# kuboyoo/alphazero-general-ori

Measured on AMD Instinct MI355X. Metric: self-play rollouts/sec (32k boards, 2p Splendor) at 1/2/4/8 MI355X, higher is better.
Workload: dtype fp32 (network) / int8 (boards) / f64 (tree statistics)

## Files before the change

### alphazero-general-ori_amd/csrc/mcts.hip

```cpp
#include <hip/hip_runtime.h>

#include <cmath>
#include <cstring>
#include <new>

#include "../../include/splendor_amd.h"

#include "board_phases.h"
#include "mcts_device.h"
#include "nn_stage.h"
#include "spl_ctx.h"

using namespace spl;

#ifndef SPL_BOUNDS_CHECK
#define SPL_BOUNDS_CHECK 0
#endif
#if SPL_BOUNDS_CHECK
__device__ unsigned long long g_bounds[4 + 64];
__device__ __noinline__ void bounds_note(int site, long long v, int t) {
    atomicAdd(&g_bounds[4 + (site & 63)], 1ull);
    if (atomicAdd(&g_bounds[0], 1ull) == 0) {
        g_bounds[1] = (unsigned long long)v; g_bounds[2] = (unsigned long long)site; g_bounds[3] = (unsigned long long)t;
    }
// ... 270 lines not shown
    for (int j = 0; j < (ec + 63) / 64; j++) {
        const int i = 64 * j + l;
        const double g = i < ec ? det_gamma(C.dir_alpha, C.seed, gb, stream, (uint32_t)i * 4096u) : 0.0;
        if (gbuf && i < ec) gbuf[i] = g;
        const int m = min(64, ec - 64 * j);
        const int lo = __double2loint(g), hi = __double2hiint(g);
        for (int k = 0; k < m; k++)
            acc = acc + __hiloint2double(__builtin_amdgcn_readlane(hi, k), __builtin_amdgcn_readlane(lo, k));
    }
    const bool ok = acc > 0.0;
    const double inv = ok ? 1.0 / acc : 0.0;
#pragma unroll 1
    for (int j = 0; j < (ec + 63) / 64; j++) {
        const int i = 64 * j + l;
        if (i < ec) {
            const int a = action_at(bits, i);
            const double g = gbuf ? gbuf[i] : (ok ? det_gamma(C.dir_alpha, C.seed, gb, stream, (uint32_t)i * 4096u) : 0.0);
            const double d = ok ? g * inv : 1.0 / (double)ec;
            pr[a] = (float)(0.75 * (double)pr[a] + 0.25 * d);
        }
    }
    wave_lds_fence();
    const float nsum = wave_np_sum409(pr);
    for (int a = l; a < SPL_ACTIONS; a += 64)
        if ((bits[a >> 6] >> (a & 63)) & 1) pr[a] = pr[a] / nsum;
    wave_lds_fence();
}

struct RunScr {
    uint64_t bits[7];
    float pr[416];
    float cp[SPL_ACTIONS];
    int16_t ca[SPL_ACTIONS];
    int16_t cvi[SPL_ACTIONS];
};

__device__ int noise_kept_root(const Pools &P, const SearchCfg &C, int t, const NodeRun &r, uint32_t stream,
                               uint64_t *bits, float *pr, float *cp, int16_t *ca, int16_t *cvi, double *gbuf = nullptr,
                               int gcap = 0) {
    const int l = lane_id();
    run_bits(P, r, bits);
    for (int a = l; a < 416; a += 64) pr[a] = 0.f;
    wave_lds_fence();
    for (int i = l; i < r.ec; i += 64) {
        const EdgeP e = *P.ep(r.eb + i);
        pr[e.a] = e.p;
        const int k = order_of(bits, e.a);
        ca[k] = e.a;
        cvi[k] = e.vi;
    }
    wave_lds_fence();
    root_noise_lds(C, t, stream, pr, bits, r.ec, gbuf, gcap);
    wave_lds_fence();
    for (int k = l; k < r.ec; k += 64) cp[k] = pr[ca[k]];
    wave_lds_fence();
    return write_sorted_run(P, r.eb, r.vb, r.ec, cp, ca, cvi);
}
__device__ __forceinline__ int noise_kept_root(const Pools &P, const SearchCfg &C, int t, const NodeRun &r,
                                               uint32_t stream, RunScr &S) {
    return noise_kept_root(P, C, t, r, stream, S.bits, S.pr, S.cp, S.ca, S.cvi);
}

#ifndef SPL_HOME_N
#define SPL_HOME_N 32
#endif
#ifndef SPL_HOME_E
#define SPL_HOME_E 24
#endif
__device__ __forceinline__ int pop_page(int32_t *stack, int32_t *top) {
    const int k = atomicSub(top, 1);
    if (k <= 0) { atomicAdd(top, 1); return -1; }
    return stack[k - 1];
}

__device__ int node_slot(const Pools &P, TreeHdr *H, int t, int id, int *npg_reg = nullptr) {
    if (id >= P.nmax) return -1;
    const int pi = id >> NPG_SHIFT;
    int32_t *tab = P.ntab + (size_t)t * P.nptab;
    if (pi >= (npg_reg ? *npg_reg : H->npg)) {
        const int pg = pi < P.nhome ? t * P.nhome + pi : pop_page(P.nfree, P.alloc + 0);
        if (pg < 0) { atomicAdd(P.alloc + 2, 1); return -1; }
        tab[pi] = pg;
        P.npidx[pg] = pi;
        H->npg = pi + 1;
        if (npg_reg) *npg_reg = pi + 1;
        return pg * NPG + (id & (NPG - 1));
    }
    return node_g(P, t, id);
}

struct AllocState {
    int64_t enext;
    int eleft, epg, edge_count;
};
__device__ __forceinline__ AllocState alloc_state(const TreeHdr *H) { return AllocState{H->enext, H->eleft, H->epg, H->edge_count}; }
__device__ int64_t unit_alloc_s(const Pools &P, TreeHdr *H, int t, int n, AllocState &a) {
    if (a.eleft < n) {
        if (a.epg >= P.eptab) return -1;
        const int pg = a.epg < P.ehome ? t * P.ehome + a.epg : pop_page(P.efree, P.alloc + 1);
        if (pg < 0) { atomicAdd(P.alloc + 3, 1); return -1; }
        P.etab[(size_t)t * P.eptab + a.epg] = pg;
        P.epidx[pg] = a.epg;
        a.epg += 1;
        H->epg = a.epg;
        a.enext = (int64_t)pg * UPG;
        a.eleft = UPG;
    }
    const int64_t b = a.enext;
    a.enext = b + n; a.eleft -= n; a.edge_count += n;
    H->enext = a.enext; H->eleft = a.eleft; H->edge_count = a.edge_count;
    return b;
}

__device__ __forceinline__ void push_pages(int32_t *stack, int32_t *top, int cap, const int32_t *tab, int from, int to,
                                           int home) {
    from = max(from, home);
    const int n = to - from;
    const int32_t *src = tab + from;
    if (n <= 0) return;
    int base = 0;
    if (lane_id() == 0) base = atomicAdd(top, n);
    base = __shfl(base, 0, 64);
    for (int i = lane_id(); i < n; i += 64)
        if (base + i < cap) stack[base + i] = src[i];
}

struct GcScr {
    int64_t *ost;
    int64_t *ovb;
    uint64_t *buf;
    int32_t *remap;
    int32_t *nvs;
    int32_t *cs;
    int32_t *cnt;
    int32_t *inv;
    int32_t *queue;
    int32_t *oec;
    int32_t *own;
};
__host__ __device__ inline size_t gc_ints(int nmax, int emax) {
    return 11 * (size_t)(nmax + 2) + 3 * (size_t)emax + 64;
}
__device__ __forceinline__ GcScr gc_scr(int32_t *base, int nmax, int emax) {
    const size_t m = (size_t)nmax + 2;
    GcScr S;
    S.ost = reinterpret_cast<int64_t *>(base);
    S.ovb = reinterpret_cast<int64_t *>(base + 2 * m);
    S.buf = reinterpret_cast<uint64_t *>(base + 4 * m);
    int32_t *q = base + 4 * m + 2 * (size_t)emax;
    S.remap = q; S.nvs = q + m; S.cs = q + 2 * m; S.cnt = q + 3 * m;
    S.inv = q + 4 * m; S.queue = q + 5 * m; S.oec = q + 6 * m; S.own = q + 7 * m;
    return S;
}

__device__ void mark_linked(const Pools &P, int t, int rootl, int32_t *mark, int32_t *q) {
    const int l = lane_id();
    const int nc = P.hdr[t].node_count;
    for (int i = l; i < nc; i += 64) mark[i] = i == rootl ? 1 : 0;
    if (l == 0) q[0] = rootl;
    wave_lds_fence();
    int head = 0, tail = 1;
    while (head < tail) {
        const int nbt = min(64, tail - head);
        int64_t vb = 0;
        int cnt = 0;
        if (l < nbt) {
            const int g = node_g(P, t, q[head + l]);
            if (!P.nd[g].h.term) {
                const NodeCold c = P.nd[g].c;
                vb = c.vb();
                cnt = c.vcnt();
            }
        }
        head += nbt;
        int incl = cnt;
#pragma unroll
        for (int o = 1; o < 64; o <<= 1) {
            const int y = __shfl_up(incl, o, 64);
            if (l >= o) incl += y;
        }
        const int tot = __shfl(incl, 63, 64), excl = incl - cnt;
        for (int c0 = 0; c0 < tot; c0 += 64) {
            const int e = c0 + l;
            int lo = 0;
#pragma unroll
            for (int step = 32; step > 0; step >>= 1)
                if (__shfl(excl, lo + step, 64) <= e) lo += step;
            const int64_t vbo = __shfl(vb, lo, 64);
            const int exo = __shfl(excl, lo, 64);
            const int c = e < tot ? P.vr(vbo + REC_UNITS * (e - exo))->child : -1;
            BCHK(c < 0 || IN_TREE(P, t, c, nc), 58, c, t, (void)0);
            const int cl = c >= 0 ? node_l(P, c) : -1;
            const bool fresh = cl >= 0 && atomicCAS(&mark[cl], 0, 1) == 0;
            const uint64_t bm = __ballot(fresh);
            if (fresh) q[tail + __popcll(bm & lanemask_lt())] = cl;
            tail += __popcll(bm);
            wave_lds_fence();
        }
    }
}

typedef uint32_t u32x4 __attribute__((ext_vector_type(4)));

constexpr int GCT = 512, GCW8 = GCT / 64;
struct GcLds {
    int32_t wsum[GCW8];
    int32_t bc[4];
};
__device__ __forceinline__ int block_scan(int x, int &total, GcLds &L) {
    const int l = lane_id(), w = threadIdx.x >> 6;
    int incl = x;
#pragma unroll
    for (int o = 1; o < 64; o <<= 1) {
        const int y = __shfl_up(incl, o, 64);
        if (l >= o) incl += y;
    }
    if (l == 63) L.wsum[w] = incl;
    __syncthreads();
    int off = 0, tot = 0;
#pragma unroll
    for (int i = 0; i < GCW8; i++) {
        const int v = L.wsum[i];
        off += i < w ? v : 0;
        tot += v;
    }
    __syncthreads();
    total = tot;
    return off + incl - x;
}

#ifndef GC_PROBE
#define GC_PROBE 0
#endif
#if GC_PROBE
constexpr int GC_WG_MAX_PROBE = 1024;
__device__ unsigned long long g_gc_probe[GC_WG_MAX_PROBE][16];
__device__ unsigned long long g_gc_probe_max[GC_WG_MAX_PROBE][8];
#define GPROBE(k)                                                                 \
    if (threadIdx.x == 0) {                                                       \
        const uint64_t c_ = __builtin_readcyclecounter();                         \
        gacc[k] += c_ - glast;                                                    \
        glast = c_;                                                               \
    }
#else
#define GPROBE(k)
#endif
constexpr int GC_NOFIT = -2;
#ifndef GC_SR
#define GC_SR 8
#endif
#ifndef GC_CR
#define GC_CR 4
#endif
template <int CR = 4>
__device__ int compact_tree(const Pools &P, int t, int root, int root_round, const GcScr &S, GcLds &L,
                            int bunits, bool linked = false) {
    const int tid = threadIdx.x;
    TreeHdr *H = P.hdr + t;
    const int nc = H->node_count;
    const int rootl = root >= 0 ? node_l(P, root) : -1;
    int32_t *remap = S.remap;
#if GC_PROBE
    uint64_t gacc[8] = {0, 0, 0, 0, 0, 0, 0, 0}, glast = __builtin_readcyclecounter();
    const uint64_t gstart = glast;
#endif
    if (linked) {
        if (tid < 64) mark_linked(P, t, rootl, remap, S.queue);
        __syncthreads();
    }
    int kept = 0;
    for (int base = 0; base < nc; base += GCT) {
        const int i = base + tid;
        bool keep = false;
        if (i < nc) keep = i == rootl || (linked ? remap[i] == 1 : P.nd[node_g(P, t, i)].h.round > root_round);
        int tot;
        const int ex = block_scan(keep ? 1 : 0, tot, L);
        if (i < nc) remap[i] = keep ? kept + ex : -1;
        kept += tot;
    }
    __syncthreads();
    GPROBE(0)
    for (int i = tid; i < nc; i += GCT) {
        int sz = -1;
        if (remap[i] >= 0) {
            sz = 0;
            const int g = node_g(P, t, i);
            const Node nd = P.nd[g];
            if (!nd.h.term) sz = nd.c.ec + REC_UNITS * nd.c.vcnt();
        }
        S.nvs[i] = sz;
    }
    __syncthreads();
    if (tid < 64) {
        const int l = tid;
        int run = 0;
        constexpr int PD = 4;
        int pre[PD];
#pragma unroll
        for (int d = 0; d < PD; d++) pre[d] = 64 * d + l < nc ? S.nvs[64 * d + l] : -1;
        for (int base = 0; base < nc; base += 64) {
            const int i = base + l;
            const int szk = pre[0];
#pragma unroll
            for (int d = 0; d + 1 < PD; d++) pre[d] = pre[d + 1];
            pre[PD - 1] = base + 64 * PD + l < nc ? S.nvs[base + 64 * PD + l] : -1;
            const bool kept = szk >= 0;
            const int sz = kept ? szk : 0;
            bool pending = sz > 0;
            int start = run;
            for (;;) {
                const int x = pending ? sz : 0;
                int incl = x;
#pragma unroll
                for (int o = 1; o < 64; o <<= 1) {
                    const int y = __shfl_up(incl, o, 64);
                    if (l >= o) incl += y;
                }
                const int st = run + incl - x;
                const bool strad = pending && (st & (UPG - 1)) + sz > UPG;
                const uint64_t m = __ballot(strad);
                if (!m) {
                    if (pending) start = st;
                    run += __shfl(incl, 63, 64);
                    break;
                }
                const int f = __ffsll((unsigned long long)m) - 1;
                if (pending && l < f) { start = st; pending = false; }
                run = (__builtin_amdgcn_readlane(st, f) & ~(UPG - 1)) + UPG;
            }
            if (kept) S.nvs[i] = start;
        }
        if (l == 0) L.bc[0] = run;
    }
    __syncthreads();
    const int run = L.bc[0];
    GPROBE(1)
    if (run > H->epg * UPG) return GC_NOFIT;
    __syncthreads();
    int my_units = 0;
    for (int base = 0; base < nc; base += GCT) {
        const int i = base + tid;
        const int ni = i < nc ? remap[i] : -1;
        uint64_t k0 = 0, k1 = 0;
        Node nd{};
        int vs = 0;
        if (ni >= 0) {
            const int g = node_g(P, t, i);
            k0 = P.nkey0[g]; k1 = P.nkey1[g];
            nd = P.nd[g];
            vs = S.nvs[i];
        }
        __syncthreads();
        if (ni >= 0) {
            const int ng = node_g(P, t, ni);
            const bool term = nd.h.term;
            const int ec = nd.c.ec, vcnt = term ? 0 : nd.c.vcnt();
            const int sz = term ? 0 : ec + REC_UNITS * vcnt;
            Node w = nd;
            S.queue[ni] = term ? -1 : nd.h.bchild;
            S.ost[ni] = nd.c.eb(); S.ovb[ni] = nd.c.vb(); S.oec[ni] = term ? 0 : ec;
            if (!term) {
                w.c.set_eb(ec > 0 ? unit_g(P, t, vs) : 0, vcnt);
                w.c.set_vb(vcnt > 0 ? unit_g(P, t, vs + ec) : 0, vcnt);
            }
            w.h.h2 = -1; w.h.h3 = -1;
            P.nkey0[ng] = k0; P.nkey1[ng] = k1;
            P.nd[ng] = w;
            S.cs[ni] = vs; S.cnt[ni] = sz; S.inv[ni] = i;
            my_units += sz;
        }
    }
    int units;
    (void)block_scan(my_units, units, L);
    GPROBE(2)
    for (int ni = tid; ni < kept; ni += GCT) {
        const int ch = S.queue[ni];
        if (ch >= 0) {
            BCHK(IN_TREE(P, t, ch, nc), 56, ((long long)ni << 32) | (uint32_t)ch, t, (void)0);
            const int nl = remap[node_l(P, ch)];
            P.nd[node_g(P, t, ni)].h.bchild = nl >= 0 ? node_g(P, t, nl) : -1;
            BCHK(nl < 0 || P.nd[node_g(P, t, nl)].h.round == P.nd[node_g(P, t, ni)].h.round + 1, 40,
                 ((long long)ni << 32) | (uint32_t)nl, t, (void)0);
        }
    }
    for (int k = tid; k < run; k += GCT) S.own[k] = -1;
    __syncthreads();
    for (int ni = tid; ni < kept; ni += GCT) {
        const int c0 = S.cs[ni], c = S.cnt[ni];
        for (int e = 0; e < c; e++) S.own[c0 + e] = ni;
    }
    __syncthreads();
    GPROBE(3)
    constexpr int SR = GC_SR;
    for (int k0 = 0; k0 < run; k0 += GCT * SR) {
        int j[SR];
#pragma unroll
        for (int r = 0; r < SR; r++) {
            const int k = k0 + GCT * r + tid;
            j[r] = k < run ? S.own[k] : -1;
        }
        int64_t src[SR];
        bool link[SR];
#pragma unroll
        for (int r = 0; r < SR; r++) {
            src[r] = 0; link[r] = false;
            if (j[r] >= 0) {
                const int rel = k0 + GCT * r + tid - S.cs[j[r]], ec = S.oec[j[r]];
                if (rel < ec) {
                    src[r] = S.ost[j[r]] + rel;
                } else {
                    const int rr = rel - ec;
                    src[r] = S.ovb[j[r]] + rr;
                    link[r] = rr % REC_UNITS == REC_LINK_UNIT;
                }
            }
        }
        uint64_t v[SR];
#pragma unroll
        for (int r = 0; r < SR; r++) v[r] = j[r] >= 0 ? P.eu[src[r]] : 0;
#pragma unroll
        for (int r = 0; r < SR; r++) {
            if (!link[r]) continue;
            const int ch = (int)(uint32_t)v[r];
            int nch = -1;
            if (ch >= 0) {
                BCHK(IN_TREE(P, t, ch, nc), 57, ((long long)j[r] << 32) | (uint32_t)ch, t, (void)0);
                const int nl = remap[node_l(P, ch)];
                if (nl >= 0) nch = node_g(P, t, nl);
                BCHK(nl < 0 || P.nd[nch].h.round == P.nd[node_g(P, t, j[r])].h.round + 1, 41,
                     ((long long)j[r] << 32) | (uint32_t)nl, t, (void)0);
            }
            v[r] = (v[r] & 0xFFFFFFFF00000000ull) | (uint64_t)(uint32_t)nch;
        }
#pragma unroll
        for (int r = 0; r < SR; r++)
            if (j[r] >= 0) S.buf[k0 + GCT * r + tid] = v[r];
    }
    __syncthreads();
    GPROBE(4)
    for (int k0 = 0; k0 < run; k0 += GCT * SR) {
        int j[SR];
        uint64_t v[SR];
#pragma unroll
        for (int r = 0; r < SR; r++) {
            const int k = k0 + GCT * r + tid;
            j[r] = k < run ? S.own[k] : -1;
            v[r] = k < run ? S.buf[k] : 0;
        }
#pragma unroll
        for (int r = 0; r < SR; r++)
            if (j[r] >= 0) P.eu[unit_g(P, t, k0 + GCT * r + tid)] = v[r];
    }
    if (P.nbrd) {
        u32x4 *bb = reinterpret_cast<u32x4 *>(P.nbrd);
        const int bu = kept * bunits;
        constexpr int R = 2 * CR;
        for (int k0 = 0; k0 < bu; k0 += GCT * R) {
            u32x4 d[R];
            size_t dst[R];
            bool mv[R];
#pragma unroll
            for (int r = 0; r < R; r++) {
                const int k = k0 + GCT * r + tid;
                mv[r] = false; dst[r] = 0; d[r] = u32x4{0, 0, 0, 0};
                if (k < bu) {
                    const int nn = k / bunits, u = k - nn * bunits, on = S.inv[nn];
                    if (on != nn) {
                        mv[r] = true;
                        dst[r] = (size_t)node_g(P, t, nn) * bunits + u;
                        d[r] = bb[(size_t)node_g(P, t, on) * bunits + u];
                    }
                }
            }
            __syncthreads();
#pragma unroll
            for (int r = 0; r < R; r++)
                if (mv[r]) bb[dst[r]] = d[r];
            __syncthreads();
        }
    }
    GPROBE(5)
    int32_t *hs = P.hslot + (size_t)t * P.hcap;
    for (int i = tid; i < P.hcap; i += GCT) hs[i] = -1;
    __syncthreads();
    for (int i = tid; i < kept; i += GCT) {
        const int g = node_g(P, t, i);
        const uint64_t k0 = P.nkey0[g];
        uint32_t h = (uint32_t)(k0 ^ (k0 >> 32)) & (uint32_t)(P.hcap - 1);
        while (atomicCAS(&hs[h], -1, g) != -1) h = (h + 1) & (uint32_t)(P.hcap - 1);
    }
    const int npg = (kept + NPG - 1) >> NPG_SHIFT, epg = (run + UPG - 1) >> UPG_SHIFT;
    const int onpg = H->npg, oepg = H->epg;
    const int nroot = rootl >= 0 && remap[rootl] >= 0 ? node_g(P, t, remap[rootl]) : -1;
    const int eleft = epg * UPG - run;
    const int64_t enext = eleft > 0 ? unit_g(P, t, run) : 0;
    __syncthreads();
    if (tid < 64) {
        push_pages(P.nfree, P.alloc + 0, P.npages, P.ntab + (size_t)t * P.nptab, npg, onpg, P.nhome);
        push_pages(P.efree, P.alloc + 1, P.epages, P.etab + (size_t)t * P.eptab, epg, oepg, P.ehome);
    }
    if (tid == 0) {
        H->node_count = kept; H->edge_count = units;
        H->npg = npg; H->epg = epg; H->eleft = eleft; H->enext = enext;
        H->live_gc = kept; H->units_gc = units; H->gcs += 1;
    }
    __syncthreads();
    GPROBE(6)
#if GC_PROBE
    if (tid == 0) {
        unsigned long long *g = g_gc_probe[blockIdx.x % GC_WG_MAX_PROBE];
        for (int k = 0; k < 7; k++) g[k] += gacc[k];
        g[8] += 1;
        const unsigned long long tot = glast - gstart;
        g[9] += tot;
        if (tot > g[10]) {
            g[10] = tot; g[11] = (unsigned long long)run; g[12] = (unsigned long long)kept; g[13] = (unsigned long long)nc;
            for (int k = 0; k < 7; k++) g_gc_probe_max[blockIdx.x % GC_WG_MAX_PROBE][k] = gacc[k];
        }
    }
#endif
    return nroot;
}

__device__ __forceinline__ long long units_used(const TreeHdr *H) { return (long long)H->epg * UPG - H->eleft; }
__device__ __forceinline__ bool tree_fits(const Pools &P, const SearchCfg &C, const TreeHdr *H) {
    return H->node_count + H->budget + 1 <= P.nmax &&
           units_used(H) + 4 * SPL_ACTIONS + (long long)H->budget * C.edge_reserve <= (long long)P.eptab * UPG;
}
__device__ void empty_tree(const Pools &P, int t) {
    TreeHdr *H = P.hdr + t;
    const int npg = H->npg, epg = H->epg;
    push_pages(P.nfree, P.alloc + 0, P.npages, P.ntab + (size_t)t * P.nptab, 0, npg, P.nhome);
    push_pages(P.efree, P.alloc + 1, P.epages, P.etab + (size_t)t * P.eptab, 0, epg, P.ehome);
    int32_t *hs = P.hslot + (size_t)t * P.hcap;
    if (H->node_count > 0 || npg > 0)
        for (int i = lane_id(); i < P.hcap; i += 64) hs[i] = -1;
    __builtin_amdgcn_wave_barrier();
    if (lane_id() == 0) {
        H->node_count = 0; H->edge_count = 0; H->npg = 0; H->epg = 0; H->eleft = 0; H->enext = 0;
        H->live_gc = 0; H->units_gc = 0;
    }
    __builtin_amdgcn_wave_barrier();
}
__device__ __forceinline__ void gc_push(const Pools &P, TreeHdr *H, int t) {
    if (H->gc_queued) return;
    H->gc_queued = 1;
    const int k = atomicAdd(&P.counters[2], 1);
    P.gcq[k] = t;
}

#ifndef GC_ALPHA_FREE
#define GC_ALPHA_FREE 8.f
#endif
template <int N>
__device__ void begin_search(const Pools &P, const SearchCfg &C, int t, const int8_t *s, bool keep,
                             bool force_full) {
    using Lx = Lay<N>;
    const int l = lane_id();
    TreeHdr *H = P.hdr + t;
    wave_store_board<N>(P.root_state + (size_t)t * Lx::S, s);
    const int mv = H->move_no;
    const bool full = force_full || philox_u01(C.seed, C.board_base + t, ST_FULL | (uint32_t)mv, 0) < C.prob_full;
    const int budget = full ? C.num_sims : C.num_sims / C.ratio_full;
    int root = -1, gcs = 0;
    const int rr = (uint8_t)bt(row(s, 0), 6);
    if (keep && H->node_count > 0) {
        uint64_t k0, k1;
        wave_fingerprint<N>(s, k0, k1);
        root = hash_lookup(P, t, k0, k1);
        BCHK(root < 0 || IN_TREE(P, t, root, H->node_count), 54, root, t, (void)0);
        const int nc = H->node_count;
        const long long used = units_used(H);
        const bool must = nc + budget + 1 > P.nmax ||
                          used + 4 * SPL_ACTIONS + (long long)budget * C.edge_reserve > (long long)P.eptab * UPG;
        const float f = fminf((float)P.alloc[0] / (float)max(P.npages - P.nhome * P.ntrees, 1),
                              (float)P.alloc[1] / (float)max(P.epages - P.ehome * P.ntrees, 1));
        const float alpha = f >= 0.75f ? GC_ALPHA_FREE : (f >= 0.5f ? 4.f : fmaxf(0.125f, 8.f * f));
        const bool should = nc > (int)((1.f + alpha) * (float)H->live_gc) + budget + NPG ||
                            used > (long long)((1.f + alpha) * (float)H->units_gc) +
                                       (long long)budget * C.edge_reserve + UPG;
        gcs = must || !C.selfplay ? 3 : (should ? 5 : 0);
    } else {
        empty_tree(P, t);
    }
    wave_lds_fence();
    if (l == 0) {
        H->root = root;
        H->sims_done = 0;
        H->full = full;
        H->budget = budget;
        H->forced = full && C.forced_playouts;
        H->noise_pending = full && C.dirichlet;
        H->leaf_kind = LEAF_NONE;
        H->overflow = 0;
        H->gc_state = gcs;
        H->root_round = rr;
        H->move_no = mv + 1;
        H->depth = 0;
        H->wd_search = 0;
        if (gcs) gc_push(P, H, t);
    }
    wave_lds_fence();
}

#ifndef GC_WG
#define GC_WG 256
#endif
#ifndef GC_SHOULD_CAP
#define GC_SHOULD_CAP GC_WG
#endif
template <int N>
__global__ __launch_bounds__(GCT) void k_gc(Pools P, SearchCfg C) {
    __shared__ GcLds L;
    __shared__ int keep_s;
    const int tid = threadIdx.x;
    const int tail = P.counters[2];
    const int ftail = P.counters[5];
    if (tail == 0 && ftail == 0) return;
    const GcScr S = gc_scr(P.gscr + (size_t)blockIdx.x * P.gc_stride, P.nmax, P.emax);
    for (int k = blockIdx.x; k < tail; k += gridDim.x) {
        const int t = P.gcq[k];
        TreeHdr *H = P.hdr + t;
        const int st = H->gc_state;
        if (tid == 0) {
            int keep = 0;
            if (st == 5 && atomicAdd(&P.counters[8], 1) >= GC_SHOULD_CAP) {
                keep = 1;
                P.gcq2[atomicAdd(&P.counters[9], 1)] = t;
            }
            keep_s = keep;
        }
        __syncthreads();
        if (keep_s) continue;
        int root = H->root;
        const int nst = st == 1 ? 2 : 0;
        if (st == 1 || st == 3 || st == 5) {
            const int rr = st == 1 && root >= 0 ? P.nd[root].h.round : H->root_round;
            const int r0 = root;
            root = compact_tree<GC_CR>(P, t, r0, rr, S, L, NodeBoard<N>::UNITS);
            bool prune = root == GC_NOFIT;
            if (!prune && st != 1) prune = !tree_fits(P, C, H) && root >= 0;
            if (prune) {
                root = compact_tree<GC_CR>(P, t, root == GC_NOFIT ? r0 : root, rr, S, L, NodeBoard<N>::UNITS, true);
                if (tid == 0) H->prunes += 1;
            }
            __syncthreads();
            if (root == GC_NOFIT || (st != 1 && !tree_fits(P, C, H))) {
                root = -1;
                if (tid < 64) empty_tree(P, t);
                if (tid == 0) H->resets += 1;
            }
        }
        __syncthreads();
        if (tid == 0) {
            H->gc_queued = 0;
            if (st == 1 || st == 3 || st == 5) {
                H->root = root;
                H->gc_state = nst;
                H->depth = 0;
            }
        }
        __syncthreads();
    }
    for (int k = blockIdx.x; k < ftail; k += gridDim.x) {
        const int2 e = P.flq[k];
        const int8_t *bs = P.ex_state + (size_t)e.x * Lay<N>::S;
        int8_t *bd = P.out_state + (size_t)e.y * Lay<N>::S;
        for (int i = tid; i < Lay<N>::S; i += GCT) bd[i] = bs[i];
        const float *src = P.ex_pi + (size_t)e.x * SPL_ACTIONS;
        float *dst = P.out_pi + (size_t)e.y * SPL_ACTIONS;
        for (int i = tid; i < SPL_ACTIONS; i += GCT) dst[i] = src[i];
    }
    __syncthreads();
    if (tid == 0) {
        __threadfence();
        keep_s = atomicAdd(&P.counters[4], 1) == (int)gridDim.x - 1;
    }
    __syncthreads();
    if (keep_s) {
        __threadfence();
        const int nk = __hip_atomic_load(&P.counters[9], __ATOMIC_RELAXED, __HIP_MEMORY_SCOPE_AGENT);
        for (int i = tid; i < nk; i += GCT)
            P.gcq[i] = __hip_atomic_load(&P.gcq2[i], __ATOMIC_RELAXED, __HIP_MEMORY_SCOPE_AGENT);
        __syncthreads();
        if (tid == 0) {
            P.counters[2] = nk;
            P.counters[5] = 0;
            P.counters[4] = 0;
            P.counters[8] = 0;
            P.counters[9] = 0;
        }
    }
}

template <int N>
__global__ __launch_bounds__(THREADS) void k_set_roots(Pools P, SearchCfg C, int B,
                                                       const int8_t *__restrict__ roots,
                                                       const uint8_t *__restrict__ active, int keep,
                                                       int force_full) {
    using Lx = Lay<N>;
    __shared__ __align__(16) int8_t lds[WAVES][Lx::LS];
    const int w = threadIdx.x >> 6, t = blockIdx.x * WAVES + w;
    if (t >= B) return;
    if (active && !active[t]) {
        if (lane_id() == 0) {
            TreeHdr *H = P.hdr + t;
            H->budget = 0; H->sims_done = 0; H->leaf_kind = LEAF_NONE;
        }
        return;
    }
    int8_t *s = lds[w];
    wave_load_board<N>(s, roots + (size_t)t * Lx::S);
    begin_search<N>(P, C, t, s, keep != 0, force_full != 0);
}

template <int N>
__device__ void deal_game(const Pools &P, const SearchCfg &C, int t, int8_t *b, double *ub) {
    TreeHdr *H = P.hdr + t;
    const int g = H->game_no;
    wave_philox_uniforms(ub, C.seed, C.board_base + (uint32_t)t, ST_DEAL | (uint32_t)g, 0, DEAL_DRAWS);
    wave_init_game<N>(b, ub);
    __threadfence_block();
    __builtin_amdgcn_wave_barrier();
    if (lane_id() == 0) {
        H->game_no = g + 1;
        H->player = 0;
        H->episode_step = 0;
        H->n_examples = 0;
    }
    __threadfence_block();
    __builtin_amdgcn_wave_barrier();
}

template <int N>
__global__ __launch_bounds__(THREADS) void k_reset_games(Pools P, SearchCfg C, int B,
                                                         const uint8_t *__restrict__ restart) {
    using Lx = Lay<N>;
    __shared__ __align__(16) int8_t lds[WAVES][Lx::LS];
    __shared__ double ub[WAVES][DEAL_DRAWS];
    const int w = threadIdx.x >> 6, t = blockIdx.x * WAVES + w;
    if (t >= B || (restart && !restart[t])) return;
    int8_t *b = lds[w];
    deal_game<N>(P, C, t, b, ub[w]);
    wave_store_board<N>(P.board + (size_t)t * Lx::S, b);
    begin_search<N>(P, C, t, b, false, false);
}

__device__ __forceinline__ long long pruned_count(long long c, int best, bool forced, float p, int sims) {
    if (forced) {
        if (c != best) c -= (long long)sqrt(0.5 * (double)p * (double)sims);
        if (c <= 1) c = 0;
    }
    return c;
}

template <int N>
__global__ __launch_bounds__(THREADS) void k_commit(Pools P, SearchCfg C, int B, int lim) {
    using Lx = Lay<N>;
    __shared__ __align__(16) int8_t lds[WAVES][2][Lx::LS];
    __shared__ double ub[WAVES][DEAL_DRAWS];
    __shared__ double pterm[WAVES][SPL_ACTIONS];
    __shared__ int16_t pact[WAVES][SPL_ACTIONS];
    __shared__ int32_t pcnt[WAVES][SPL_ACTIONS];
    __shared__ __align__(16) float pprior[WAVES][SPL_ACTIONS + 3];
    __shared__ uint64_t pbits[WAVES][7];
    const int w = threadIdx.x >> 6, t = blockIdx.x * WAVES + w;
    if (t >= B) return;
    const int l = lane_id();
    TreeHdr *H = P.hdr + t;
    if (H->gc_state == 1 || H->sims_done < H->budget || H->overflow || H->root < 0) return;
    const uint32_t gb = C.board_base + (uint32_t)t;
    const int root = H->root;
    const NodeRun rr = run_of(P.nd[root].c);
    const int ec = rr.ec;
    const bool forced = H->forced;
    const int sims = H->budget, cm = H->move_no;
    run_bits(P, rr, pbits[w]);
    int best = 0;
    for (int i = l; i < ec; i += 64) {
        const EdgeP e = *P.ep(rr.eb + i);
        const int n = e.vi >= 0 ? P.vr(rr.vb + REC_UNITS * e.vi)->n : 0;
        const int k = order_of(pbits[w], e.a);
        pact[w][k] = e.a; pcnt[w][k] = n; pprior[w][k] = e.p;
        best = max(best, n);
    }
    best = wave_max_i32(best);
    wave_lds_fence();
    int mode = forced ? 0 : 1;
    long long tot = 0;
    for (; mode < 3; mode++) {
        tot = 0;
        for (int i = l; i < ec; i += 64)
            tot += mode == 0 ? pruned_count(pcnt[w][i], best, true, pprior[w][i], sims) : (mode == 1 ? pcnt[w][i] : 1);
        for (int o = 32; o > 0; o >>= 1) tot += __shfl_xor(tot, o, 64);
        if (tot > 0) break;
    }
#define POLICY_COUNT(i) (mode == 0 ? pruned_count(pcnt[w][i], best, true, pprior[w][i], sims) : (mode == 1 ? (long long)pcnt[w][i] : 1ll))
    const int step = H->episode_step + 1;
    const int player = H->player;
    int8_t *s = lds[w][0], *b = lds[w][1];
    int nex = H->n_examples;
    if (H->full && nex < P.excap) {
        const size_t x = (size_t)t * P.excap + nex;
        wave_load_board<N>(s, P.root_state + (size_t)t * Lx::S);
        wave_store_board<N>(P.ex_state + x * Lx::S, s);
        float *pi = P.ex_pi + x * SPL_ACTIONS;
        for (int a = l; a < SPL_ACTIONS; a += 64) pi[a] = 0.f;
        __threadfence_block();
        __builtin_amdgcn_wave_barrier();
        for (int i = l; i < ec; i += 64)
            pi[pact[w][i]] = (float)((double)POLICY_COUNT(i) / (double)tot);
        uint64_t m[7];
        wave_valid_moves<N>(s, 0, lim, m);
        store_mask(P.ex_valid + x * 7, m);
        if (l == 0) {
            const double q0 = P.nd[root].h.qs;
            P.ex_player[x] = player;
            for (int i = 0; i < 4; i++)
                P.ex_q[x * 4 + i] = i == 0 ? (float)q0 : (i < N ? (float)(-q0 / (double)(N - 1)) : 0.f);
        }
        nex++;
    }
    int action = 408;
    const double T = C.temp_threshold > 0 ? (step < C.temp_threshold ? 2.0 : 0.2) : 1.0;
    for (int i = l; i < ec; i += 64) pterm[w][i] = temp_pow((double)POLICY_COUNT(i) / (double)tot, T);
    __threadfence_block();
    __builtin_amdgcn_wave_barrier();
    double sum = 0.0;
    if (l == 0) {
        const double *pt = pterm[w];
        for (int i = 0; i < ec; i++) sum += pt[i];
    }
    sum = readlane_f64(sum, 0);
    for (int i = l; i < ec; i += 64) pterm[w][i] = pterm[w][i] / sum;
    __threadfence_block();
    __builtin_amdgcn_wave_barrier();
    if (l == 0) {
        double *pt = pterm[w];
        double cdf = 0.0;
        for (int i = 0; i < ec; i++) {
            cdf += pt[i];
// ... 1717 lines not shown
#endif

#if GC_PROBE
int spl_diag_gc_probe(unsigned long long *out24, int reset) {
    static unsigned long long h[GC_WG_MAX_PROBE][16], hm[GC_WG_MAX_PROBE][8];
    if (hipMemcpyFromSymbol(h, HIP_SYMBOL(g_gc_probe), sizeof(h)) != hipSuccess) return SPL_EDEVICE;
    if (hipMemcpyFromSymbol(hm, HIP_SYMBOL(g_gc_probe_max), sizeof(hm)) != hipSuccess) return SPL_EDEVICE;
    for (int k = 0; k < 24; k++) out24[k] = 0;
    for (int i = 0; i < GC_WG_MAX_PROBE; i++) {
        for (int k = 0; k < 10; k++) out24[k] += h[i][k];
        if (h[i][10] > out24[10]) {
            for (int k = 10; k < 14; k++) out24[k] = h[i][k];
            for (int k = 0; k < 7; k++) out24[16 + k] = hm[i][k];
        }
    }
    if (reset) {
        memset(h, 0, sizeof(h));
        memset(hm, 0, sizeof(hm));
        if (hipMemcpyToSymbol(HIP_SYMBOL(g_gc_probe), h, sizeof(h)) != hipSuccess) return SPL_EDEVICE;
        if (hipMemcpyToSymbol(HIP_SYMBOL(g_gc_probe_max), hm, sizeof(hm)) != hipSuccess) return SPL_EDEVICE;
    }
    return 0;
}
#endif

#if LM_PROBE
int spl_diag_lm_probe(unsigned long long *out) {
    return hipMemcpyFromSymbol(out, HIP_SYMBOL(g_lm_probe), sizeof(g_lm_probe)) == hipSuccess ? 0 : SPL_EDEVICE;
}
#endif

#if BACKUP_PROBE
int spl_diag_backup_probe(unsigned long long *out16, int reset) {
    static unsigned long long h[BK_PSLOTS][16];
    if (hipMemcpyFromSymbol(h, HIP_SYMBOL(g_bk_probe), sizeof(h)) != hipSuccess) return SPL_EDEVICE;
    for (int k = 0; k < 16; k++) out16[k] = 0;
    for (int i = 0; i < BK_PSLOTS; i++)
        for (int k = 0; k < 16; k++) out16[k] += h[i][k];
    if (reset) {
        memset(h, 0, sizeof(h));
        if (hipMemcpyToSymbol(HIP_SYMBOL(g_bk_probe), h, sizeof(h)) != hipSuccess) return SPL_EDEVICE;
    }
    return 0;
}
#endif

#if SPL_BOUNDS_CHECK
int spl_diag_bounds(unsigned long long *out4, int reset) {
    if (hipMemcpyFromSymbol(out4, HIP_SYMBOL(g_bounds), 68 * 8) != hipSuccess) return SPL_EDEVICE;
    if (reset) {
        unsigned long long z[68] = {0};
        if (hipMemcpyToSymbol(HIP_SYMBOL(g_bounds), z, sizeof(z)) != hipSuccess) return SPL_EDEVICE;
    }
    return 0;
}
#endif

long long spl_mcts_plan_bytes(const spl_ctx *ctx, int B, const spl_mcts_config *cfg) {
    if (!valid_cfg(ctx, B, cfg)) return SPL_EINVAL;
    return (long long)plan_pools(ctx->n, B, cfg).bytes;
}

int spl_mcts_create(const spl_ctx *ctx, int B, const spl_mcts_config *cfg, spl_mcts **out) {
    if (!valid_cfg(ctx, B, cfg) || !out) return SPL_EINVAL;
    spl_mcts *m = new (std::nothrow) spl_mcts;
    if (!m) return SPL_EINVAL;
    m->n = ctx->n; m->B = B; m->S = 7 * (32 + 10 * ctx->n + ctx->n * ctx->n);
    m->token_limit = ctx->token_limit;
    m->rules = ctx->rules;
    SearchCfg &C = m->cfg;
    C.cpuct = cfg->cpuct; C.fpu = cfg->fpu; C.dir_alpha = cfg->dirichlet_alpha;
    C.dir_temp = cfg->dirichlet_temp > 0 ? cfg->dirichlet_temp : 1.0;
    C.prob_full = cfg->prob_full; C.num_sims = cfg->num_sims; C.ratio_full = cfg->ratio_full;
    C.forced_playouts = cfg->forced_playouts; C.dirichlet = cfg->dirichlet_alpha > 0;
    C.temp_threshold = cfg->temp_threshold; C.seed = cfg->seed; C.board_base = cfg->board_base;
    C.selfplay = cfg->selfplay;
    C.edge_reserve = 48;
    Pools &P = m->P;
    const Plan L = plan_pools(ctx->n, B, cfg);
    P.nmax = L.nmax; P.emax = L.emax; P.hcap = L.hcap; P.pcap = L.pcap;
    P.nptab = L.nptab; P.eptab = L.eptab;
    P.npages = (int)L.npages; P.epages = (int)L.epages;
    P.ntrees = B;
    P.nhome = min(min(SPL_HOME_N, P.nptab), (int)(L.npages / (4 * (long long)B)));
    while (P.nhome & (P.nhome - 1)) P.nhome &= P.nhome - 1;
    P.ehome = min(min(SPL_HOME_E, P.eptab), (int)(L.epages / (4 * (long long)B)));
    const size_t nn = (size_t)L.npages * NPG, ne = (size_t)L.epages * UPG;
    const int excap = L.excap;
    const size_t nx = (size_t)B * excap, no = (size_t)L.out_cap;
    const int gcw = B < GC_WG ? B : GC_WG;
    void *arena = nullptr;
    if (hipMalloc(&arena, L.bytes) != hipSuccess) { delete m; return SPL_EDEVICE; }
    m->arena = arena;
    m->bytes = L.bytes;
    char *p = (char *)arena;
    P.hdr = carve<TreeHdr>(p, B);
    P.nkey0 = carve<uint64_t>(p, nn); P.nkey1 = carve<uint64_t>(p, nn);
    P.nd = carve<Node>(p, nn);
    P.eu = carve<uint64_t>(p, ne);
    P.ntab = carve<int32_t>(p, (size_t)B * P.nptab); P.etab = carve<int32_t>(p, (size_t)B * P.eptab);
    P.npidx = carve<int32_t>(p, (size_t)P.npages); P.epidx = carve<int32_t>(p, (size_t)P.epages);
    P.nfree = carve<int32_t>(p, (size_t)P.npages); P.efree = carve<int32_t>(p, (size_t)P.epages);
    P.alloc = carve<int32_t>(p, 16);
    P.hslot = carve<int32_t>(p, (size_t)B * P.hcap);
    P.path_n = carve<int32_t>(p, (size_t)B * (P.pcap + 1));
    P.path_x = carve<int32_t>(p, (size_t)B * P.pcap);
    P.path_b = carve<int64_t>(p, (size_t)B * P.pcap);
    P.gc_stride = gc_ints(P.nmax, P.emax);
    P.gscr = carve<int32_t>(p, (size_t)gcw * P.gc_stride);
    P.root_state = carve<int8_t>(p, (size_t)B * m->S);
    P.excap = excap; P.out_cap = (int)no;
    P.board = carve<int8_t>(p, (size_t)B * m->S);
    P.ex_state = carve<int8_t>(p, nx * m->S); P.ex_pi = carve<float>(p, nx * SPL_ACTIONS);
    P.ex_q = carve<float>(p, 4 * nx); P.ex_valid = carve<uint64_t>(p, 7 * nx);
    P.ex_player = carve<int32_t>(p, nx);
    P.out_state = carve<int8_t>(p, no * m->S); P.out_pi = carve<float>(p, no * SPL_ACTIONS);
    P.out_winner = carve<float>(p, 4 * no); P.out_q = carve<float>(p, 4 * no);
    P.out_valid = carve<uint64_t>(p, 7 * no); P.out_scdiff = carve<int32_t>(p, 4 * no);
    P.out_meta = carve<int32_t>(p, 4 * no); P.counters = carve<int32_t>(p, 16);
    P.nbrd = L.nbb ? carve<int8_t>(p, (size_t)L.nbb * nn) : nullptr;
    P.gcq = carve<int32_t>(p, (size_t)B);
    P.gcq2 = carve<int32_t>(p, (size_t)B);
    P.flq = carve<int2>(p, no);
    bool ok = hipMemset(P.hdr, 0, sizeof(TreeHdr) * B) == hipSuccess &&
              hipMemset(P.counters, 0, 64) == hipSuccess &&
              hipMemset(P.hslot, 0xFF, 4 * (size_t)B * P.hcap) == hipSuccess;
    if (ok) {
        hipLaunchKernelGGL(k_init_pools, dim3(1024), dim3(256), 0, (hipStream_t)0, P, B);
        ok = hipGetLastError() == hipSuccess && hipDeviceSynchronize() == hipSuccess;
    }
    if (!ok) { (void)hipFree(arena); delete m; return SPL_EDEVICE; }
    *out = m;
    return 0;
}

int spl_mcts_destroy(spl_mcts *m) {
    if (!m) return 0;
    (void)hipFree(m->arena);
    delete m;
    return 0;
}

long long spl_mcts_device_bytes(const spl_mcts *m) {
    if (!m) return SPL_EINVAL;
    return (long long)m->bytes;
}

int spl_mcts_rules(const spl_mcts *m) { return m ? m->rules : SPL_EINVAL; }

int spl_mcts_set_roots(spl_mcts *m, const int8_t *roots, int keep_tree, int force_full, void *hs) {
    return spl_mcts_set_roots_active(m, roots, nullptr, keep_tree, force_full, hs);
}

static void launch_gc(spl_mcts *m, hipStream_t hs) {
    const unsigned gcw = (unsigned)(m->B < GC_WG ? m->B : GC_WG);
    SPL_DISPATCH(m->n, hipLaunchKernelGGL(k_gc<N>, dim3(gcw), dim3(GCT), 0, hs, m->P, m->cfg));
}

int spl_mcts_set_roots_active(spl_mcts *m, const int8_t *roots, const uint8_t *active, int keep_tree,
                              int force_full, void *hs) {
    if (!m || !roots) return SPL_EINVAL;
    SPL_DISPATCH(m->n, hipLaunchKernelGGL(k_set_roots<N>, wave_grid(m->B), dim3(THREADS), 0,
                                          (hipStream_t)hs, m->P, m->cfg, m->B, roots, active, keep_tree,
                                          force_full));
    launch_gc(m, (hipStream_t)hs);
    return check_launch();
}

int spl_mcts_pick_best(spl_mcts *m, const uint8_t *active, uint32_t board_base, uint32_t stream,
                       int16_t *action, void *hs) {
    if (!m || !action || stream > 0xFFFFFFu) return SPL_EINVAL;
    hipLaunchKernelGGL(k_pick_best, wave_grid(m->B), dim3(THREADS), 0, (hipStream_t)hs, m->P, m->cfg,
                       m->B, active, board_base, stream, action);
    return check_launch();
}

static int launch_select(spl_mcts *m, int8_t *leaf_state, uint64_t *leaf_mask, uint8_t *leaf_valid,
                         int32_t *leaf_index, int32_t *leaf_count, void *hs) {
    SPL_DISPATCH(m->n, hipLaunchKernelGGL(k_select_lanes<N>, dim3((unsigned)((m->B + 63) / 64)), dim3(64), 0,
                                          (hipStream_t)hs, m->P, m->cfg, m->B, mcts_lim(m),
                                          leaf_state, leaf_valid));
    char *no_stage = nullptr;
    SPL_DISPATCH(m->n, hipLaunchKernelGGL(k_leaf_mask<N>, dim3((unsigned)((m->B + 63) / 64)), dim3(256), 0,
                                          (hipStream_t)hs, m->P, m->B, mcts_lim(m), leaf_state, leaf_valid,
                                          leaf_mask, leaf_index, leaf_count, no_stage));
    return check_launch();
}

static int launch_mask_staged(int n, const Pools &P, int B, int lim, const int8_t *leaf_state,
                              const uint8_t *leaf_valid, uint64_t *leaf_mask, void *stage, void *hs) {
    int32_t *no_list = nullptr;
    char *st = static_cast<char *>(stage);
    SPL_DISPATCH(n, hipLaunchKernelGGL((k_leaf_mask<N, true>), dim3((unsigned)((B + 63) / 64)), dim3(256), 0,
                                       (hipStream_t)hs, P, B, lim, leaf_state, leaf_valid, leaf_mask, no_list,
                                       no_list, st));
    return check_launch();
}
static bool stage_args_ok(const void *leaf_state, const void *leaf_mask, const void *leaf_valid, const void *stage) {
    return leaf_state && leaf_mask && leaf_valid && stage && reinterpret_cast<uintptr_t>(leaf_state) % 4 == 0 &&
           reinterpret_cast<uintptr_t>(leaf_mask) % 8 == 0 && reinterpret_cast<uintptr_t>(leaf_valid) % 16 == 0 &&
           reinterpret_cast<uintptr_t>(stage) % 16 == 0;
}

int spl_mcts_select_staged(spl_mcts *m, int8_t *leaf_state, uint64_t *leaf_mask, uint8_t *leaf_valid, void *stage,
                           void *hs) {
    if (!m || !stage_args_ok(leaf_state, leaf_mask, leaf_valid, stage)) return SPL_EINVAL;
    SPL_DISPATCH(m->n, hipLaunchKernelGGL(k_select_lanes<N>, dim3((unsigned)((m->B + 63) / 64)), dim3(64), 0,
                                          (hipStream_t)hs, m->P, m->cfg, m->B, mcts_lim(m),
                                          leaf_state, leaf_valid));
    return launch_mask_staged(m->n, m->P, m->B, mcts_lim(m), leaf_state, leaf_valid, leaf_mask, stage, hs);
}

int spl_nn_stage_leaves(const spl_ctx *ctx, int B, const int8_t *leaf_state, const uint8_t *leaf_valid,
                        uint64_t *leaf_mask, void *stage, void *hs) {
    if (!ok_ctx(ctx) || B < 0 || !stage_args_ok(leaf_state, leaf_mask, leaf_valid, stage))
        return SPL_EINVAL;
    if (!B) return 0;
    return launch_mask_staged(ctx->n, Pools{}, B, pack_lim(ctx->token_limit, ctx->rules), leaf_state, leaf_valid,
                              leaf_mask, stage, hs);
}

int spl_mcts_select(spl_mcts *m, int8_t *leaf_state, uint64_t *leaf_mask, uint8_t *leaf_valid,
                    void *hs) {
    if (!m || !leaf_state || !leaf_mask || !leaf_valid) return SPL_EINVAL;
    return launch_select(m, leaf_state, leaf_mask, leaf_valid, nullptr, nullptr, hs);
}

int spl_mcts_select_compact(spl_mcts *m, int8_t *leaf_state, uint64_t *leaf_mask, uint8_t *leaf_valid,
                            int32_t *leaf_index, int32_t *leaf_count, void *hs) {
    if (!m || !leaf_state || !leaf_mask || !leaf_valid || !leaf_index || !leaf_count) return SPL_EINVAL;
    return launch_select(m, leaf_state, leaf_mask, leaf_valid, leaf_index, leaf_count, hs);
}

int spl_mcts_backup_kind(spl_mcts *m, const uint64_t *leaf_mask, const float *pi, const float *v, int kinds,
                         void *hs) {
    const bool defer_gc = (kinds & SPL_BACKUP_DEFER_GC) != 0;
    kinds &= ~SPL_BACKUP_DEFER_GC;
    if (!m || kinds < 1 || kinds > 3 || ((kinds & SPL_LEAF_NN) && (!leaf_mask || !pi || !v))) return SPL_EINVAL;
    const dim3 grid = wave_grid((m->B + 1) / 2);
    if (kinds == 3) {
        SPL_DISPATCH(m->n, hipLaunchKernelGGL((k_backup_h<N, 3>), grid, dim3(THREADS), 0, (hipStream_t)hs, m->P,
                                              m->cfg, m->B, leaf_mask, pi, v));
    } else if (kinds == SPL_LEAF_NN) {
        SPL_DISPATCH(m->n, hipLaunchKernelGGL((k_backup_h<N, 1>), grid, dim3(THREADS), 0, (hipStream_t)hs, m->P,
                                              m->cfg, m->B, leaf_mask, pi, v));
    } else {
        SPL_DISPATCH(m->n, hipLaunchKernelGGL((k_backup_h<N, 2>), grid, dim3(THREADS), 0, (hipStream_t)hs, m->P,
                                              m->cfg, m->B, leaf_mask, pi, v));
    }
    if (m->cfg.selfplay && (kinds & SPL_LEAF_NN) && !defer_gc) launch_gc(m, (hipStream_t)hs);
    return check_launch();
}

int spl_mcts_backup(spl_mcts *m, const uint64_t *leaf_mask, const float *pi, const float *v,
                    void *hs) {
    if (!m || !leaf_mask || !pi || !v) return SPL_EINVAL;
    return spl_mcts_backup_kind(m, leaf_mask, pi, v, 3, hs);
}

int spl_mcts_root_stats(spl_mcts *m, int64_t *counts, double *qsa, double *probs, double *q,
                        int64_t *adjusted, void *hs) {
    if (!m) return SPL_EINVAL;
    hipLaunchKernelGGL(k_root_stats, wave_grid(m->B), dim3(THREADS), 0, (hipStream_t)hs, m->P,
                       m->cfg, m->B, m->n, counts, qsa, probs, q, adjusted);
    return check_launch();
}

int spl_mcts_root_priors(spl_mcts *m, float *ps, void *hs) {
    if (!m || !ps) return SPL_EINVAL;
    hipLaunchKernelGGL(k_root_priors, wave_grid(m->B), dim3(THREADS), 0, (hipStream_t)hs, m->P, m->B, ps);
    return check_launch();
}

int spl_mcts_reset_games(spl_mcts *m, void *hs) {
    if (!m || !m->cfg.selfplay) return SPL_EINVAL;
    SPL_DISPATCH(m->n, hipLaunchKernelGGL(k_reset_games<N>, wave_grid(m->B), dim3(THREADS), 0,
                                          (hipStream_t)hs, m->P, m->cfg, m->B, nullptr));
    return check_launch();
}

int spl_mcts_restart_games(spl_mcts *m, const uint8_t *restart, void *hs) {
    if (!m || !m->cfg.selfplay || !restart) return SPL_EINVAL;
    SPL_DISPATCH(m->n, hipLaunchKernelGGL(k_reset_games<N>, wave_grid(m->B), dim3(THREADS), 0,
                                          (hipStream_t)hs, m->P, m->cfg, m->B, restart));
    return check_launch();
}

int spl_mcts_commit(spl_mcts *m, void *hs) {
    if (!m || !m->cfg.selfplay) return SPL_EINVAL;
    SPL_DISPATCH(m->n, hipLaunchKernelGGL(k_commit<N>, wave_grid(m->B), dim3(THREADS), 0,
                                          (hipStream_t)hs, m->P, m->cfg, m->B, mcts_lim(m)));
    launch_gc(m, (hipStream_t)hs);
    return check_launch();
}

int spl_mcts_drain_examples(spl_mcts *m, int8_t *state, float *pi, uint64_t *valid, float *winner,
                            int32_t *scdiff, float *q, int32_t *meta, int max, int32_t *n_out,
                            void *hs) {
    if (!m || !m->cfg.selfplay || max < 0) return SPL_EINVAL;
    const size_t work = (size_t)(max < m->P.out_cap ? max : m->P.out_cap) * SPL_ACTIONS / 4;
    if (work) {
        const unsigned grid = (unsigned)((work + 255) / 256 > 8192 ? 8192 : (work + 255) / 256);
        hipLaunchKernelGGL(k_drain_copy, dim3(grid), dim3(256), 0, (hipStream_t)hs, m->P, m->S, max,
                           state, pi, valid, winner, scdiff, q, meta, m->n);
    }
    hipLaunchKernelGGL(k_drain_reset, dim3(1), dim3(1), 0, (hipStream_t)hs, m->P, max, n_out);
    return check_launch();
}

// ... 57 lines not shown
```

Measured before the change: 75.97 million.

## Stage GC compaction scratch in LDS arena and use dynamic work-stealing over trees

The tree garbage-collection kernel now carves its per-tree scratch arrays (remap, sizes, queues, offsets, buffers) out of a roughly 160KB LDS arena when the tree is small enough, and falls back to global scratch otherwise. Trees are handed out through an atomic counter instead of a static grid-stride loop, the deferral cap is raised to 1024, and node records are moved as raw 64-byte vectors. The intent is to cut global-memory traffic and load imbalance in GC. The large LDS footprint limits occupancy to one workgroup per CU, and new diagnostic counters add a few atomics.

```diff
diff --git a/alphazero-general-ori_amd/csrc/mcts.hip b/alphazero-general-ori_amd/csrc/mcts.hip
--- a/alphazero-general-ori_amd/csrc/mcts.hip
+++ b/alphazero-general-ori_amd/csrc/mcts.hip
@@ -446,6 +446,22 @@
     S.inv = q + 4 * m; S.queue = q + 5 * m; S.oec = q + 6 * m; S.own = q + 7 * m;
     return S;
 }
+constexpr int GC_LDS_INTS = 40448;
+struct GcArena {
+    int32_t *p;
+    int left;
+    __device__ __forceinline__ int32_t *take(int ints, int32_t *fallback) {
+        ints = (ints + 1) & ~1;
+        if (ints > left) return fallback;
+        int32_t *r = p;
+        p += ints; left -= ints;
+        return r;
+    }
+};
+__host__ __device__ inline int gc_lds_nodes(int limit) {
+    const int cap = GC_LDS_INTS / 2 - 2;
+    return limit < 0 || limit > cap ? cap : limit;
+}
 
 __device__ void mark_linked(const Pools &P, int t, int rootl, int32_t *mark, int32_t *q) {
     const int l = lane_id();
@@ -495,6 +511,22 @@
 }
 
 typedef uint32_t u32x4 __attribute__((ext_vector_type(4)));
+struct NodeRaw {
+    u32x4 q[4];
+    __device__ __forceinline__ int bchild() const { return (int)q[0].x; }
+    __device__ __forceinline__ bool term() const { return (q[1].y & 0xFFu) != 0; }
+    __device__ __forceinline__ uint64_t ebq() const { return (uint64_t)q[2].x | ((uint64_t)q[2].y << 32); }
+    __device__ __forceinline__ uint64_t vbq() const { return (uint64_t)q[2].z | ((uint64_t)q[2].w << 32); }
+    __device__ __forceinline__ int ec() const { return (int)(int16_t)(q[3].x & 0xFFFFu); }
+    __device__ __forceinline__ void set_runs(uint64_t e, uint64_t v) {
+        q[2] = u32x4{(uint32_t)e, (uint32_t)(e >> 32), (uint32_t)v, (uint32_t)(v >> 32)};
+    }
+    __device__ __forceinline__ void clear_hints() { q[0].y = 0xFFFFFFFFu; q[0].z = 0xFFFFFFFFu; }
+};
+static_assert(sizeof(NodeRaw) == sizeof(Node) && offsetof(Node, h.bchild) == 0 && offsetof(Node, h.h2) == 4 &&
+                  offsetof(Node, h.h3) == 8 && offsetof(Node, h.term) == 20 && offsetof(Node, c.ebq) == 32 &&
+                  offsetof(Node, c.vbq) == 40 && offsetof(Node, c.ec) == 48,
+              "NodeRaw's field offsets");
 
 constexpr int GCT = 512, GCW8 = GCT / 64;
 struct GcLds {
@@ -547,12 +579,17 @@
 #define GC_CR 4
 #endif
 template <int CR = 4>
-__device__ int compact_tree(const Pools &P, int t, int root, int root_round, const GcScr &S, GcLds &L,
-                            int bunits, bool linked = false) {
+__device__ int compact_tree(const Pools &P, int t, int root, int root_round, const GcScr &G, int32_t *lds,
+                            int lds_nodes, GcLds &L, int bunits, bool linked = false) {
     const int tid = threadIdx.x;
     TreeHdr *H = P.hdr + t;
     const int nc = H->node_count;
     const int rootl = root >= 0 ? node_l(P, root) : -1;
+    GcScr S = G;
+    GcArena A{lds, nc <= lds_nodes ? GC_LDS_INTS : 0};
+    S.remap = A.take(nc, G.remap);
+    S.nvs = A.take(nc, G.nvs);
+    if (linked) S.queue = A.take(nc, G.queue);
     int32_t *remap = S.remap;
 #if GC_PROBE
     uint64_t gacc[8] = {0, 0, 0, 0, 0, 0, 0, 0}, glast = __builtin_readcyclecounter();
@@ -573,6 +610,11 @@
         kept += tot;
     }
     __syncthreads();
+    S.cs = A.take(kept, G.cs); S.oec = A.take(kept, G.oec);
+    S.ost = reinterpret_cast<int64_t *>(A.take(2 * kept, reinterpret_cast<int32_t *>(G.ost)));
+    S.ovb = reinterpret_cast<int64_t *>(A.take(2 * kept, reinterpret_cast<int32_t *>(G.ovb)));
+    S.cnt = A.take(kept, G.cnt); S.inv = A.take(kept, G.inv);
+    if (!linked) S.queue = A.take(kept, G.queue);
     GPROBE(0)
     for (int i = tid; i < nc; i += GCT) {
         int sz = -1;
@@ -631,35 +673,42 @@
     GPROBE(1)
     if (run > H->epg * UPG) return GC_NOFIT;
     __syncthreads();
+    S.own = A.take(run, G.own);
+    S.buf = reinterpret_cast<uint64_t *>(A.take(2 * run, reinterpret_cast<int32_t *>(G.buf)));
     int my_units = 0;
     for (int base = 0; base < nc; base += GCT) {
         const int i = base + tid;
         const int ni = i < nc ? remap[i] : -1;
         uint64_t k0 = 0, k1 = 0;
-        Node nd{};
+        NodeRaw nd{};
         int vs = 0;
         if (ni >= 0) {
             const int g = node_g(P, t, i);
+            vs = S.nvs[i];
             k0 = P.nkey0[g]; k1 = P.nkey1[g];
-            nd = P.nd[g];
-            vs = S.nvs[i];
+            nd = *reinterpret_cast<const NodeRaw *>(P.nd + g);
         }
         __syncthreads();
         if (ni >= 0) {
             const int ng = node_g(P, t, ni);
-            const bool term = nd.h.term;
-            const int ec = nd.c.ec, vcnt = term ? 0 : nd.c.vcnt();
+            const bool term = nd.term();
+            const uint64_t ebq = nd.ebq(), vbq = nd.vbq();
+            const int ec = nd.ec(), vcnt = term ? 0 : (int)(vbq >> 48);
             const int sz = term ? 0 : ec + REC_UNITS * vcnt;
-            Node w = nd;
-            S.queue[ni] = term ? -1 : nd.h.bchild;
-            S.ost[ni] = nd.c.eb(); S.ovb[ni] = nd.c.vb(); S.oec[ni] = term ? 0 : ec;
+            NodeRaw w = nd;
+            const int bch = term ? -1 : nd.bchild();
+            const int64_t oeb = (int64_t)(ebq & LOW48), ovb = (int64_t)(vbq & LOW48);
             if (!term) {
-                w.c.set_eb(ec > 0 ? unit_g(P, t, vs) : 0, vcnt);
-                w.c.set_vb(vcnt > 0 ? unit_g(P, t, vs + ec) : 0, vcnt);
+                NodeCold c;
+                c.set_eb(ec > 0 ? unit_g(P, t, vs) : 0, vcnt);
+                c.set_vb(vcnt > 0 ? unit_g(P, t, vs + ec) : 0, vcnt);
+                w.set_runs(c.ebq, c.vbq);
             }
-            w.h.h2 = -1; w.h.h3 = -1;
+            w.clear_hints();
             P.nkey0[ng] = k0; P.nkey1[ng] = k1;
-            P.nd[ng] = w;
+            *reinterpret_cast<NodeRaw *>(P.nd + ng) = w;
+            S.queue[ni] = bch;
+            S.ost[ni] = oeb; S.ovb[ni] = ovb; S.oec[ni] = term ? 0 : ec;
             S.cs[ni] = vs; S.cnt[ni] = sz; S.inv[ni] = i;
             my_units += sz;
         }
@@ -901,41 +950,56 @@
 #define GC_WG 256
 #endif
 #ifndef GC_SHOULD_CAP
-#define GC_SHOULD_CAP GC_WG
-#endif
+#define GC_SHOULD_CAP 1024
+#endif
+__device__ unsigned long long g_gc_paths[4];
 template <int N>
-__global__ __launch_bounds__(GCT) void k_gc(Pools P, SearchCfg C) {
+__global__ __launch_bounds__(GCT) void k_gc(Pools P, SearchCfg C, int lds_limit) {
+    __shared__ __align__(16) int32_t arena[GC_LDS_INTS];
     __shared__ GcLds L;
-    __shared__ int keep_s;
+    __shared__ int keep_s, pop_s;
     const int tid = threadIdx.x;
     const int tail = P.counters[2];
     const int ftail = P.counters[5];
     if (tail == 0 && ftail == 0) return;
     const GcScr S = gc_scr(P.gscr + (size_t)blockIdx.x * P.gc_stride, P.nmax, P.emax);
-    for (int k = blockIdx.x; k < tail; k += gridDim.x) {
+    const int lds_nodes = gc_lds_nodes(lds_limit);
+    int taken = 0;
+    for (;;) {
+        if (tid == 0) {
+            const int k = atomicAdd(&P.counters[6], 1);
+            int keep = 0;
+            if (k < tail) {
+                const int t = P.gcq[k];
+                if (P.hdr[t].gc_state == 5 && atomicAdd(&P.counters[8], 1) >= GC_SHOULD_CAP) {
+                    keep = 1;
+                    P.gcq2[atomicAdd(&P.counters[9], 1)] = t;
+                }
+            }
+            pop_s = k; keep_s = keep;
+        }
+        __syncthreads();
+        const int k = pop_s;
+        const bool deferred = keep_s != 0;
+        __syncthreads();
+        if (k >= tail) break;
+        taken++;
+        if (deferred) continue;
         const int t = P.gcq[k];
         TreeHdr *H = P.hdr + t;
         const int st = H->gc_state;
-        if (tid == 0) {
-            int keep = 0;
-            if (st == 5 && atomicAdd(&P.counters[8], 1) >= GC_SHOULD_CAP) {
-                keep = 1;
-                P.gcq2[atomicAdd(&P.counters[9], 1)] = t;
-            }
-            keep_s = keep;
-        }
-        __syncthreads();
-        if (keep_s) continue;
         int root = H->root;
         const int nst = st == 1 ? 2 : 0;
         if (st == 1 || st == 3 || st == 5) {
+            if (tid == 0) atomicAdd(&g_gc_paths[H->node_count <= lds_nodes ? 0 : 1], 1ull);
             const int rr = st == 1 && root >= 0 ? P.nd[root].h.round : H->root_round;
             const int r0 = root;
-            root = compact_tree<GC_CR>(P, t, r0, rr, S, L, NodeBoard<N>::UNITS);
+            root = compact_tree<GC_CR>(P, t, r0, rr, S, arena, lds_nodes, L, NodeBoard<N>::UNITS);
             bool prune = root == GC_NOFIT;
             if (!prune && st != 1) prune = !tree_fits(P, C, H) && root >= 0;
             if (prune) {
-                root = compact_tree<GC_CR>(P, t, root == GC_NOFIT ? r0 : root, rr, S, L, NodeBoard<N>::UNITS, true);
+                root = compact_tree<GC_CR>(P, t, root == GC_NOFIT ? r0 : root, rr, S, arena, lds_nodes, L,
+                                           NodeBoard<N>::UNITS, true);
                 if (tid == 0) H->prunes += 1;
             }
             __syncthreads();
@@ -956,6 +1020,7 @@
         }
         __syncthreads();
     }
+    if (tid == 0 && taken > 0) atomicMax(&g_gc_paths[2], (unsigned long long)taken);
     for (int k = blockIdx.x; k < ftail; k += gridDim.x) {
         const int2 e = P.flq[k];
         const int8_t *bs = P.ex_state + (size_t)e.x * Lay<N>::S;
@@ -978,9 +1043,11 @@
             P.gcq[i] = __hip_atomic_load(&P.gcq2[i], __ATOMIC_RELAXED, __HIP_MEMORY_SCOPE_AGENT);
         __syncthreads();
         if (tid == 0) {
+            if (tail > 0) g_gc_paths[3] += 1;
             P.counters[2] = nk;
             P.counters[5] = 0;
             P.counters[4] = 0;
+            P.counters[6] = 0;
             P.counters[8] = 0;
             P.counters[9] = 0;
         }
@@ -3004,9 +3071,24 @@
     return spl_mcts_set_roots_active(m, roots, nullptr, keep_tree, force_full, hs);
 }
 
+static int g_gc_lds_limit = -1;
 static void launch_gc(spl_mcts *m, hipStream_t hs) {
     const unsigned gcw = (unsigned)(m->B < GC_WG ? m->B : GC_WG);
-    SPL_DISPATCH(m->n, hipLaunchKernelGGL(k_gc<N>, dim3(gcw), dim3(GCT), 0, hs, m->P, m->cfg));
+    SPL_DISPATCH(m->n, hipLaunchKernelGGL(k_gc<N>, dim3(gcw), dim3(GCT), 0, hs, m->P, m->cfg, g_gc_lds_limit));
+}
+
+extern "C" int spl_diag_gc_paths(unsigned long long *out4, int reset) {
+    if (!out4 || hipMemcpyFromSymbol(out4, HIP_SYMBOL(g_gc_paths), 4 * 8) != hipSuccess) return SPL_EDEVICE;
+    if (reset) {
+        unsigned long long z[4] = {0, 0, 0, 0};
+        if (hipMemcpyToSymbol(HIP_SYMBOL(g_gc_paths), z, sizeof(z)) != hipSuccess) return SPL_EDEVICE;
+    }
+    return 0;
+}
+extern "C" int spl_diag_gc_lds_limit(int nodes) {
+    const int prev = g_gc_lds_limit;
+    g_gc_lds_limit = nodes < 0 ? -1 : nodes;
+    return prev;
 }
 
 int spl_mcts_set_roots_active(spl_mcts *m, const int8_t *roots, const uint8_t *active, int keep_tree,
```

After: 77.71 million (median of 6 runs). +2.3%, better.
